# PROBIC/mSWEEP

Measured on AMD Instinct MI355X. Metric: EM iters/sec + reads×groups cells/sec, 10M reads × 5k groups, higher is better.
Workload: dtype f64

## Files before the change

### msweep_amd/csrc/host_likelihood.inc

```
namespace {

void sell_from_device(msw_core *h, const uint32_t *d_rowptr, const uint32_t *d_grp, const uint32_t *d_idx,
                      const double *cell_val = nullptr);
bool compress_dense(msw_core *h, const double *Lm, size_t ld, const double *stage, size_t G, size_t E, bool force);

}

void msw::host::reset_likelihood(msw_core *h) {
  Resident &L = h->lik;
  static_cast<LikShape &>(L) = LikShape{};
  h->solver.have_solution = false;
  h->solver.prepared = false;
  h->iperm.release();
  h->assign.drop();
  L.long_row = multilane() ? kLongRow : kLongRowOneLane;
  if (const char *lr = getenv("MSWEEP_LONG_ROW"))
    L.long_row = (uint32_t)std::min(std::max(atoi(lr), 16), (int)L.long_row);
}

namespace {

constexpr uint8_t kRGroup[64] = {0, 0, 0, 0, 1, 1, 1, 1, 1, 1, 1, 1, 0, 0, 0, 0, 1, 1, 1, 1, 0, 0,
                                 0, 0, 0, 0, 0, 0, 1, 1, 1, 1, 2, 2, 2, 2, 3, 3, 3, 3, 3, 3, 3, 3,
                                 2, 2, 2, 2, 3, 3, 3, 3, 2, 2, 2, 2, 2, 2, 2, 2, 3, 3, 3, 3};

constexpr uint8_t kRPos[64] = {0, 1, 2,  3,  0,  1,  2,  3,  4,  5,  6,  7,  4,  5,  6,  7,  8,  9,  10, 11, 8, 9,
                               10, 11, 12, 13, 14, 15, 12, 13, 14, 15, 0,  1,  2,  3,  0,  1,  2,  3,  4,  5, 6, 7,
                               4,  5,  6,  7,  8,  9,  10, 11, 8,  9,  10, 11, 12, 13, 14, 15, 12, 13, 14, 15};

struct SlotPlan {
  std::vector<uint32_t> canon, hot_rank;
  uint32_t rep_base = 0, H = 0, sentinel_slot = 0;
};
SlotPlan plan_slot_area(msw_core *h, const std::vector<uint64_t> &freq) {
  Resident &L = h->lik;
  const uint32_t n_lut = L.n_lut;
  SlotPlan sp;
  std::vector<uint32_t> used;
  for (uint32_t i = 0; i < n_lut; ++i) if (freq[i]) used.push_back(i);
  if (used.empty()) used.push_back(0);
  std::vector<uint32_t> by_freq(used);
  std::stable_sort(by_freq.begin(), by_freq.end(), [&](uint32_t a, uint32_t b) { return freq[a] > freq[b]; });
  sp.canon.assign(std::max<uint32_t>(n_lut, 1), 0);
  sp.hot_rank.assign(std::max<uint32_t>(n_lut, 1), UINT32_MAX);
  sp.sentinel_slot = used[0];
  for (uint32_t tryH : {64u, 32u, 16u, 8u, 0u}) {
    if (tryH > used.size()) continue;
    sp.H = tryH;
    sp.rep_base = sp.H ? (uint32_t)((used.size() + 15) & ~(size_t)15) : (uint32_t)used.size();
    L.n_area = sp.rep_base + 8 * sp.H;
    choose_layout(L);
    if (L.tlds && L.glds && !L.wide()) break;
  }
  bool hybrid = false;
  if (!L.tlds) {
    sp.H = 0;
    sp.rep_base = (uint32_t)used.size();
    L.n_area = (uint32_t)used.size();
    choose_layout(L);
    hybrid = choose_hybrid_layout(L, h->no_hybrid);
    if (hybrid) sp.sentinel_slot = by_freq[0];
  }
  const std::vector<uint32_t> &order = hybrid ? by_freq : used;
  std::vector<uint32_t> area_slot(L.n_area, used[0]);
  for (uint32_t e = 0; e < order.size(); ++e) area_slot[e] = order[e], sp.canon[order[e]] = e;
  for (uint32_t j = 0; j < sp.H; ++j) {
    sp.hot_rank[by_freq[j]] = j;
    for (uint32_t c = 0; c < 8; ++c) area_slot[sp.rep_base + (j >> 1) * 16 + 2 * c + (j & 1)] = by_freq[j];
  }
  L.area_slot.upload(area_slot.data(), area_slot.size(), h->stream);
  L.lut_area.alloc(L.n_area);
  hipLaunchKernelGGL(k_gather_f64, dim3((L.n_area + 255) / 256), dim3(256), 0, h->stream, L.lut.p, L.area_slot.p,
                     L.n_area, L.lut_area.p);
  L.trange.alloc(2);
  minmax_launch(1, h->stream, L.lut_area.p, (uint64_t)L.n_area, 0, L.trange.p);
  MSW_HIP(hipGetLastError());
  MSW_HIP(hipStreamSynchronize(h->stream));
  return sp;
}

void finish_sell(msw_core *h) {
  Resident &L = h->lik;
  const uint32_t wg_for_slices = (L.nslices + (kPassThreads / 64) - 1) / (kPassThreads / 64);
  L.nblk = (int)std::max<uint32_t>(1, std::min<uint32_t>(std::max(wg_for_slices, L.n_long), (uint32_t)h->n_cu));
  L.nblk_dense = 0;
  L.flavor = 0;
  L.packed_scheduled = h->pack_schedule;
  L.rows_over8 = 0;
  L.passB_rc8 = false;
  if (L.nslices && L.enc == kEncNarrow && L.cls.s0[kSliceClasses - 1] == 0) {
    DevBuf<unsigned long long> d_over;
    d_over.alloc(1);
    d_over.zero(h->stream);
    hipLaunchKernelGGL(k_rows_over, dim3(std::min<uint32_t>((L.nslices + 255) / 256, (uint32_t)h->n_cu * 8)), dim3(256), 0,
                       h->stream, L.slice_off.p, L.nslices, 8u, d_over.p);
    unsigned long long over = 0;
    MSW_HIP(hipMemcpyAsync(&over, d_over.p, sizeof over, hipMemcpyDeviceToHost, h->stream));
    MSW_HIP(hipStreamSynchronize(h->stream));
    L.rows_over8 = over;
    L.passB_rc8 = 20 * over <= L.nslots / 64;
    if (const char *e = getenv("MSWEEP_PASSB_RC")) L.passB_rc8 = atoi(e) == 8;
  }
  alloc_solve_state(L, h->solver);
  MSW_HIP(hipStreamSynchronize(h->stream));
}

template <class RP>
void upload_sell(msw_core *h, const RP *rowptr, const uint32_t *cell_grp, const uint32_t *cell_idx) {
  Resident &L = h->lik;
  const uint32_t E = L.E, G = L.G, n_lut = L.n_lut;
  const uint64_t nnz_all = rowptr[E];
  std::vector<uint64_t> freq(std::max<uint32_t>(n_lut, 1), 0);
  for (uint64_t k = 0; k < nnz_all; ++k) ++freq[cell_idx[k]];
  const SlotPlan sp = plan_slot_area(h, freq);
  const std::vector<uint32_t> &canon = sp.canon, &hot_rank = sp.hot_rank;
  const uint32_t rep_base = sp.rep_base;
  const std::vector<uint32_t> used = {sp.sentinel_slot};
  const bool wide = L.wide(), hybrid = L.hybrid();
  const int rw = wide ? 2 : 1;
  const RecDec dec = L.dec;
  const uint32_t n_hot = L.n_tab_lds;
  auto entry_of = [&](int lane, uint32_t idx) -> uint32_t {
    const uint32_t j = hot_rank[idx];
    if (lane < 0 || j == UINT32_MAX) return canon[idx];
    return rep_base + (j >> 1) * 16 + 2 * (kRPos[lane] >> 1) + (j & 1);
  };
  auto put_entry = [&](std::vector<uint32_t> &dst, size_t slot, uint32_t g, uint32_t entry, bool hot = false) {
    if (wide) {
      const uint2 r = Rec<kEncWide>::make(g, entry, dec);
      dst[2 * slot] = r.x;
      dst[2 * slot + 1] = r.y;
    } else if (hybrid) {
      dst[slot] = hot ? Rec<kEncIndex>::make_h(g, entry, dec) : Rec<kEncIndex>::make(g, entry, dec);
    } else {
      dst[slot] = Rec<kEncNarrow>::make(g, entry, dec);
    }
  };
  auto put = [&](std::vector<uint32_t> &dst, size_t slot, uint32_t g, uint32_t idx, int lane, bool hot = false) {
    put_entry(dst, slot, g, entry_of(lane, idx), hot);
  };
  std::vector<uint32_t> perm(E);
  std::vector<uint32_t> cnt_len((kLongRow + 2) * 4, 0);
  std::vector<uint8_t> ccls(E, 0);
  uint32_t n_long = 0;
  uint32_t n_class[kSliceClasses] = {};
  const bool ml = multilane();
  for (uint32_t j = 0; j < E; ++j) {
    const uint64_t len = rowptr[j + 1] - rowptr[j];
    if (hybrid && len <= 16) {
      uint32_t cc = 0;
      for (uint64_t k = rowptr[j]; k < rowptr[j + 1]; ++k) cc += canon[cell_idx[k]] >= n_hot;
      ccls[j] = (uint8_t)cold_class(cc);
    }
    if (len > (uint64_t)L.long_row) {
      ++n_long;
    } else {
      ++cnt_len[len * 4 + ccls[j]];
      ++n_class[slice_class_of((uint32_t)len, ml)];
    }
  }
  {
    std::vector<uint32_t> start((kLongRow + 2) * 4, 0);
    uint32_t pos = n_long;
    for (int len = kLongRow; len >= 0; --len)
      for (int cl = 0; cl < 4; ++cl) {
        start[len * 4 + cl] = pos;
        pos += cnt_len[len * 4 + cl];
      }
    uint32_t pl = 0;
    for (uint32_t j = 0; j < E; ++j) {
      const uint64_t len = rowptr[j + 1] - rowptr[j];
      if (len > (uint64_t)L.long_row) perm[pl++] = j;
      else perm[start[len * 4 + ccls[j]]++] = j;
    }
  }
  std::vector<uint32_t> long_ptr(n_long + 1, 0);
  for (uint32_t p = 0; p < n_long; ++p)
    long_ptr[p + 1] = long_ptr[p] + (uint32_t)(rowptr[perm[p] + 1] - rowptr[perm[p]]);
  std::vector<uint32_t> rec_long((size_t)long_ptr[n_long] * rw + 2);
  for (uint32_t p = 0; p < n_long; ++p) {
    const uint64_t b = rowptr[perm[p]];
    const uint32_t n = long_ptr[p + 1] - long_ptr[p];
    uint32_t cnt[kLongResidues] = {}, run[kLongResidues] = {};
    for (uint32_t k = 0; k < n; ++k) ++cnt[cell_grp[b + k] & (kLongResidues - 1)];
    for (uint32_t k = 0; k < n; ++k) {
      const uint32_t r = cell_grp[b + k] & (kLongResidues - 1);
      put(rec_long, (size_t)long_ptr[p] + long_cell_pos(cnt, r, run[r]++), cell_grp[b + k], cell_idx[b + k], -1);
    }
  }
  L.cls = make_slice_classes(n_class);
  const SliceClasses cls = L.cls;
  const bool schedule = h->pack_schedule;
  const uint32_t nslices = cls.s0[kSliceClasses];
  std::vector<uint32_t> slice_off(nslices + 1, 0);
  for (uint32_t s = 0; s < nslices; ++s) {
    const SliceGeo sg = slice_geo(cls, s);
    const uint32_t j0 = perm[n_long + (size_t)sg.ec0];
    const uint64_t len0 = rowptr[j0 + 1] - rowptr[j0];
    uint64_t maxlen = (len0 + (1u << sg.lgm) - 1) >> sg.lgm;
    if (!odd_slices(L.enc)) maxlen += maxlen & 1;
    const uint64_t nxt = (uint64_t)slice_off[s] + maxlen;
    if (nxt > 0xffffffffull) throw Fail("msw_core_set_csr: likelihood too large for 32-bit slice offsets");
    slice_off[s + 1] = (uint32_t)nxt;
  }
  if (hybrid && slice_off[nslices] >= (1u << kGeoHotShift))
    throw Fail("msw_core_set_csr: likelihood too large for the hybrid slot area's slice geometry");
  const size_t nslots = (size_t)slice_off[nslices] * 64;
  std::vector<uint32_t> rec((nslots + 64) * rw + 2);
  std::vector<uint8_t> slice_hot(hybrid ? nslices : 0, 0);
  {
    const int nthr = std::max(1u, std::min(32u, std::thread::hardware_concurrency()));
    std::vector<std::thread> pool;
    for (int t = 0; t < nthr; ++t) {
      pool.emplace_back([&, t] {
        std::vector<uint64_t> cells;
        std::vector<uint32_t> centry;
        std::vector<uint32_t> cbeg(65);
        std::vector<uint8_t> ctaken;
        for (uint32_t s = t; s < nslices; s += nthr) {
          const uint32_t len = slice_off[s + 1] - slice_off[s];
          const size_t base = (size_t)slice_off[s] * 64;
          cells.clear();
          centry.clear();
          const SliceGeo sg = slice_geo(cls, s);
          const uint32_t m = 1u << sg.lgm;
          for (int l = 0; l < 64; ++l) {
            cbeg[l] = (uint32_t)cells.size();
            if (((uint32_t)l >> sg.lgm) < sg.nec) {
              const uint32_t j = perm[n_long + sg.ec0 + ((uint32_t)l >> sg.lgm)];
              for (uint64_t k = rowptr[j] + ((uint32_t)l & (m - 1)); k < rowptr[j + 1]; k += m) {
                cells.push_back(((uint64_t)cell_grp[k] << 32) | cell_idx[k]);
                centry.push_back(entry_of(l, cell_idx[k]));
              }
            }
          }
          cbeg[64] = (uint32_t)cells.size();
          ctaken.assign(cells.size(), 0);
          const bool streaming = len > 16;
          for (uint32_t k0 = 0; k0 < len; k0 += 16) {
            const uint32_t nrows = std::min<uint32_t>(16, len - k0);
            uint32_t wb[64], we[64];
            for (int l = 0; l < 64; ++l) {
              wb[l] = std::min(cbeg[l] + k0, cbeg[l + 1]);
              we[l] = std::min(wb[l] + 16, cbeg[l + 1]);
            }
            uint32_t nhot = nrows;
            if (hybrid && !streaming) {
              uint32_t mc = 0;
              for (int l = 0; l < 64; ++l) {
                uint32_t cc = 0;
                for (uint32_t c = wb[l]; c < we[l]; ++c) cc += centry[c] >= n_hot;
                mc = std::max(mc, cc);
              }
              nhot = mc > (uint32_t)kColdRows ? 0u : len - mc;
              slice_hot[s] = (uint8_t)nhot;
            }
            for (uint32_t k = 0; k < nhot; ++k) {
              uint32_t rg[4][16], rs[4][16], hg[2][32];
              uint16_t at[4] = {0, 0, 0, 0};
              std::memset(rg, 0xff, sizeof rg);
              std::memset(rs, 0xff, sizeof rs);
              std::memset(hg, 0xff, sizeof hg);
              for (int li = 0; li < 64; ++li) {
                const int l = (li + (int)(k0 + k) * 7) & 63;
                const int R = kRGroup[l], C = l >> 4, H = l >> 5;
                const size_t slot = base + (size_t)(k0 + k) * 64 + l;
                int best = -1, best_score = -1;
                for (uint32_t c = wb[l]; c < we[l]; ++c) {
                  if (ctaken[c]) continue;
                  const uint32_t g = (uint32_t)(cells[c] >> 32), i = centry[c];
                  if (hybrid && !streaming && i >= n_hot) continue;
                  int score = 0;
                  if (!(at[C] >> (g & 15) & 1)) score += MSW_W_AT;
                  if (rg[R][g & 15] == UINT32_MAX || rg[R][g & 15] == g) score += MSW_W_EW;
                  if (rs[R][i & 15] == UINT32_MAX || rs[R][i & 15] == i) score += MSW_W_XT;
                  if (hg[H][g & 31] == UINT32_MAX || hg[H][g & 31] == g) score += MSW_W_E;
                  if (!schedule) score = MSW_W_AT + MSW_W_EW + MSW_W_XT + MSW_W_E;
                  if (score > best_score) {
                    best_score = score;
                    best = (int)c;
                    if (score == MSW_W_AT + MSW_W_EW + MSW_W_XT + MSW_W_E) break;
                  }
                }
                const bool hot_row = hybrid && !streaming;
                if (best < 0) {
                  put(rec, slot, G + (uint32_t)l, used[0], -1, hot_row);
                  continue;
                }
                ctaken[best] = 1;
                const uint32_t g = (uint32_t)(cells[best] >> 32), i = centry[best];
                at[C] |= (uint16_t)(1u << (g & 15));
                if (rg[R][g & 15] == UINT32_MAX) rg[R][g & 15] = g;
                if (rs[R][i & 15] == UINT32_MAX) rs[R][i & 15] = i;
                if (hg[H][g & 31] == UINT32_MAX) hg[H][g & 31] = g;
                put(rec, slot, g, (uint32_t)cells[best], l, hot_row);
              }
            }
            for (int l = 0; l < 64; ++l) {
              uint32_t c = wb[l];
              for (uint32_t k = nhot; k < nrows; ++k) {
                const size_t slot = base + (size_t)(k0 + k) * 64 + l;
                while (c < we[l] && ctaken[c]) ++c;
                if (c < we[l]) {
                  put_entry(rec, slot, (uint32_t)(cells[c] >> 32), centry[c]);
                  ++c;
                } else {
                  put(rec, slot, G + (uint32_t)l, used[0], -1);
                }
              }
            }
          }
        }
      });
    }
    for (auto &th : pool) th.join();
  }
  if (getenv("MSW_DEBUG_SCHED")) {
    uint64_t steps = 0, cyc_ew = 0, cyc_xt = 0, cyc_at = 0, cyc_e = 0;
    for (uint32_t s = 0; s < nslices; ++s) {
      const uint32_t len = slice_off[s + 1] - slice_off[s];
      const size_t base = (size_t)slice_off[s] * 64;
      for (uint32_t k = 0; k < len; ++k) {
        uint32_t vg[64], vi[64];
        for (int l = 0; l < 64; ++l) {
          const size_t slot = base + (size_t)k * 64 + l;
          if (wide) {
            const uint2 r = make_uint2(rec[2 * slot], rec[2 * slot + 1]);
            vg[l] = Rec<kEncWide>::grp(r, dec), vi[l] = Rec<kEncWide>::t_off(r, dec) >> 4;
          } else if (hybrid) {
            const bool hot = k < slice_hot[s];
            vg[l] = hot ? Rec<kEncIndex>::grp_h(rec[slot], dec) : Rec<kEncIndex>::grp(rec[slot], dec);
            vi[l] = (hot ? Rec<kEncIndex>::t_off_h(rec[slot], dec) : Rec<kEncIndex>::t_off(rec[slot], dec)) >> 4;
          } else {
            vg[l] = Rec<kEncNarrow>::grp(rec[slot], dec), vi[l] = Rec<kEncNarrow>::t_off(rec[slot], dec) >> 4;
          }
        }
        auto cyc = [&](const uint32_t *v, int ngroups, auto group_of, uint32_t nbanks, bool combine) {
          int total = 0;
          for (int gr = 0; gr < ngroups; ++gr) {
            int mx = 0;
            for (uint32_t bnk = 0; bnk < nbanks; ++bnk) {
              uint32_t seen[64]; int ns = 0;
              for (int l = 0; l < 64; ++l) if (group_of(l) == gr && (v[l] % nbanks) == bnk) {
                bool dup = false;
                if (combine) for (int q = 0; q < ns; ++q) dup |= seen[q] == v[l];
                if (!dup) seen[ns++] = v[l];
              }
              mx = std::max(mx, ns);
            }
            total += mx;
          }
          return total;
        };
        ++steps;
        cyc_ew += cyc(vg, 4, [](int l) { return (int)kRGroup[l]; }, 16, true);
        cyc_xt += cyc(vi, 4, [](int l) { return (int)kRGroup[l]; }, 16, true);
        cyc_at += cyc(vg, 4, [](int l) { return l >> 4; }, 16, false);
        cyc_e += cyc(vg, 2, [](int l) { return l >> 5; }, 32, true);
      }
    }
    fprintf(stderr, "[msw sched] steps %llu  modelled LDS cycles / wave instruction: {e,w} b128 %.2f (ideal 4)  "
                    "slot b128 %.2f (4)  atomics %.2f (4)  e_g b64 %.2f (2)\n",
            (unsigned long long)steps, (double)cyc_ew / steps, (double)cyc_xt / steps, (double)cyc_at / steps,
            (double)cyc_e / steps);
  }
  L.n_long = n_long;
  L.nslices = nslices;
  L.nslots = nslots;
  L.perm.upload(perm.data(), perm.size(), h->stream);
  L.long_ptr.upload(long_ptr.data(), long_ptr.size(), h->stream);
  L.rec_long.upload(rec_long.data(), rec_long.size(), h->stream);
  L.slice_off.upload(slice_off.data(), slice_off.size(), h->stream);
  L.rec.upload(rec.data(), rec.size(), h->stream);
  if (hybrid) L.slice_hot.upload(slice_hot.data(), std::max<size_t>(slice_hot.size(), 1), h->stream);
  finish_sell(h);
}

void set_csr_impl(msw_core *h, const uint64_t *rowptr, const uint32_t *grp, const uint32_t *cnt,
                  const double *lut, size_t lut_ld, double logzi, size_t G, size_t E) {
  Resident &L = h->lik;
// ... 208 lines not shown
```

### msweep_amd/csrc/host_pack.inc

```
namespace {

uint64_t device_scan_u32(msw_core *h, uint32_t *d, uint64_t n, DevBuf<uint32_t> &tot, DevBuf<uint64_t> &gt);

void choose_value_layout(Resident &L) {
  L.enc = kEncValue;
  L.tlds = false;
  L.n_area = 0;
  L.n_tab_lds = 0;
  L.dec.shift = 0;
  L.dec.mask = 0;
  L.dec.bhi = L.dec.bhiA = 0;
  const char *force = getenv("MSWEEP_FORCE_LDS");
  const bool want_glds = !(force && strlen(force) == 2 && force[0] == '0');
  L.glds = want_glds && pass_lds_bytes(1, 0, L.G, true, false) <= kLdsMax && passB_mode(L, true, 0, false) >= 0;
  L.gmodeB = passB_mode(L, L.glds, 0, false);
  if (L.gmodeB < 0) throw Fail("internal: no LDS configuration fits");
  if (8ull * ((uint64_t)L.G + kSentinels) >= (1ull << 31)) throw Fail("likelihood too large: group offsets exceed the record field");
}

void sell_from_device(msw_core *h, const uint32_t *d_rowptr, const uint32_t *d_grp, const uint32_t *d_idx,
                      const double *cell_val ) {
  Resident &L = h->lik;
  const uint32_t E = L.E, n_lut = L.n_lut;
  const uint64_t nnz = L.nnz;
// ... 25 lines not shown
    const size_t lds = n_lut <= 16384 ? (size_t)n_lut * sizeof(unsigned int) : 0;
    hipLaunchKernelGGL(k_slot_hist, dim3((unsigned)std::min<uint64_t>((nnz + 4095) / 4096, (uint64_t)h->n_cu * 8)), dim3(256),
                       lds, st, d_idx, nnz, n_lut, d_freq.p);
  }
  std::vector<unsigned long long> f(std::max<uint32_t>(n_lut, 1), 0);
  MSW_HIP(hipMemcpyAsync(f.data(), d_freq.p, f.size() * sizeof(unsigned long long), hipMemcpyDeviceToHost, st));
  MSW_HIP(hipStreamSynchronize(st));
  const std::vector<uint64_t> freq(f.begin(), f.end());
  sp = plan_slot_area(h, freq);
  d_canon.upload(sp.canon.data(), sp.canon.size(), st);
  d_hot.upload(sp.hot_rank.data(), sp.hot_rank.size(), st);
  }
  tm.mark("  pack: slot plan");
  DevBuf<uint32_t> key, key2, val, cnt;
  key.alloc(E);
  key2.alloc(E);
  val.alloc(E);
  L.perm.alloc(E);
  cnt.alloc(1 + kSliceClasses);
  MSW_HIP(hipMemsetAsync(cnt.p, 0, (1 + kSliceClasses) * sizeof(uint32_t), st));
  const unsigned nbe = (unsigned)std::min<size_t>(((size_t)E + 255) / 256, (size_t)h->n_cu * 16);
  hipLaunchKernelGGL(k_pack_keys, dim3(nbe), dim3(256), 0, st, d_rowptr, E, L.long_row, multilane() ? 1 : 0, d_idx,
                     L.hybrid() ? d_canon.p : (const uint32_t *)nullptr, L.n_tab_lds, key.p, val.p, cnt.p);
  size_t tmp_bytes = 0;
  MSW_HIP(prim_sort_pairs(nullptr, tmp_bytes, key.p, key2.p, val.p, L.perm.p, (size_t)E, kPackKeyBits, st));
  DevBuf<unsigned char> tmp;
  tmp.alloc(tmp_bytes);
  MSW_HIP(prim_sort_pairs(tmp.p, tmp_bytes, key.p, key2.p, val.p, L.perm.p, (size_t)E, kPackKeyBits, st));
  uint32_t counts[1 + kSliceClasses] = {};
  MSW_HIP(hipMemcpyAsync(counts, cnt.p, sizeof counts, hipMemcpyDeviceToHost, st));
  MSW_HIP(hipStreamSynchronize(st));
  tm.mark("  pack: keys + sort");
  const uint32_t n_long = counts[0];
  const uint32_t n_sell = E - n_long;
  L.cls = make_slice_classes(counts + 1);
  const uint32_t nslices = L.cls.s0[kSliceClasses];
  L.long_ptr.alloc((size_t)n_long + 1);
  L.slice_off.alloc((size_t)nslices + 1);
  MSW_HIP(hipMemsetAsync(L.long_ptr.p, 0, ((size_t)n_long + 1) * sizeof(uint32_t), st));
  MSW_HIP(hipMemsetAsync(L.slice_off.p, 0, ((size_t)nslices + 1) * sizeof(uint32_t), st));
  const uint32_t nmax = std::max(n_long, nslices);
  if (nmax)
    hipLaunchKernelGGL(k_pack_lens, dim3((nmax + 255) / 256), dim3(256), 0, st, d_rowptr, L.perm.p, n_long, nslices,
                       odd_slices(L.enc) ? 0 : 1, L.cls, L.long_ptr.p, L.slice_off.p);
  DevBuf<uint32_t> tot;
  DevBuf<uint64_t> gt;
  const uint64_t n_long_cells = device_scan_u32(h, L.long_ptr.p, (uint64_t)n_long + 1, tot, gt);
  const uint64_t n_rows = device_scan_u32(h, L.slice_off.p, (uint64_t)nslices + 1, tot, gt);
  if (n_rows > 0xffffffffull || n_long_cells > 0xffffffffull)
    throw Fail("msw_core_set_csr: likelihood too large for 32-bit slice offsets");
  uint64_t hyb_rows_max = 1ull << kGeoHotShift;
  if (const char *e = getenv("MSWEEP_HYBRID_MAX_ROWS")) hyb_rows_max = std::min<uint64_t>(hyb_rows_max, strtoull(e, nullptr, 10));
  if (L.hybrid() && n_rows >= hyb_rows_max) {
    if (h->no_hybrid) throw Fail("msw_core_set_csr: likelihood too large for the hybrid slot area's slice geometry");
    h->no_hybrid = true;
    try {
      sell_from_device(h, d_rowptr, d_grp, d_idx, cell_val);
    } catch (...) {
      h->no_hybrid = false;
      throw;
    }
    h->no_hybrid = false;
    return;
  }
  const size_t nslots = (size_t)n_rows * 64;
  if (L.hybrid()) L.slice_hot.alloc(std::max<uint32_t>(nslices, 1));
  L.rec.alloc(rec_words(L.enc, nslots + 64) + 2);
  L.rec_long.alloc(rec_words(L.enc, (size_t)n_long_cells + 64) + 2);
  MSW_HIP(hipMemsetAsync(L.rec.p + rec_words(L.enc, nslots), 0, (rec_words(L.enc, 64) + 2) * sizeof(uint32_t), st));
  MSW_HIP(hipMemsetAsync(L.rec_long.p, 0, (rec_words(L.enc, (size_t)n_long_cells + 64) + 2) * sizeof(uint32_t), st));
  tm.mark("  pack: geometry + alloc");
  const PackEnc pe{d_canon.p, d_hot.p, sp.rep_base, L.G, sp.sentinel_slot, L.dec, L.n_tab_lds, L.slice_hot.p,
                   cell_val, L.logzi};
  if (n_long) {
    auto k = L.enc == kEncValue ? k_pack_long<kEncValue>
                                 : (L.wide() ? k_pack_long<kEncWide> : (L.hybrid() ? k_pack_long<kEncIndex> : k_pack_long<kEncNarrow>));
    hipLaunchKernelGGL(k, dim3(std::min<uint32_t>(n_long, (uint32_t)h->n_cu * 32)), dim3(64), 0, st, d_rowptr, d_grp, d_idx,
                       L.perm.p, L.long_ptr.p, n_long, pe, L.rec_long.p);
  }
  if (nslices) {
    auto k = L.enc == kEncValue ? k_pack_slices<kEncValue>
                                 : (L.wide() ? k_pack_slices<kEncWide> : (L.hybrid() ? k_pack_slices<kEncIndex> : k_pack_slices<kEncNarrow>));
    hipLaunchKernelGGL(k, dim3(std::min<uint32_t>(nslices, (uint32_t)h->n_cu * 64)), dim3(64), 0, st, d_rowptr, d_grp,
                       d_idx, L.perm.p, L.slice_off.p, n_long, n_sell, nslices, L.cls, pe, h->pack_schedule ? 1 : 0, L.rec.p);
  }
  MSW_HIP(hipGetLastError());
  tm.mark("  pack: records");
  L.n_long = n_long;
  L.nslices = nslices;
  L.nslots = nslots;
  finish_sell(h);
  tm.mark("  pack: solver state");
}

uint64_t layout_hash(const Resident &L) {
  if (L.flavor != 0) throw Fail("msw_core_layout_hash: no CSR-of-ECs likelihood resident");
  uint64_t hash = 1469598103934665603ull;
  auto eat = [&](const uint32_t *d, size_t n) {
    std::vector<uint32_t> v(n);
    if (n) MSW_HIP(hipMemcpy(v.data(), d, n * sizeof(uint32_t), hipMemcpyDeviceToHost));
    const unsigned char *p = reinterpret_cast<const unsigned char *>(v.data());
    for (size_t i = 0; i < n * 4; ++i) hash = (hash ^ p[i]) * 1099511628211ull;
  };
  std::vector<uint32_t> lp(L.n_long + 1);
  MSW_HIP(hipMemcpy(lp.data(), L.long_ptr.p, lp.size() * sizeof(uint32_t), hipMemcpyDeviceToHost));
  eat(L.perm.p, L.E);
  eat(L.slice_off.p, (size_t)L.nslices + 1);
  eat(L.long_ptr.p, (size_t)L.n_long + 1);
  eat(L.rec.p, rec_words(L.enc, L.nslots));
  eat(L.rec_long.p, rec_words(L.enc, (size_t)lp[L.n_long]));
  eat(L.area_slot.p, L.n_area);
  for (int c = 0; c <= kSliceClasses; ++c) {
    const uint32_t w[2] = {L.cls.s0[c], L.cls.p0[c]};
    const unsigned char *pb = reinterpret_cast<const unsigned char *>(w);
    for (size_t i = 0; i < sizeof w; ++i) hash = (hash ^ pb[i]) * 1099511628211ull;
  }
  if (L.hybrid()) {
    std::vector<uint8_t> sh(L.nslices);
    if (L.nslices) MSW_HIP(hipMemcpy(sh.data(), L.slice_hot.p, L.nslices, hipMemcpyDeviceToHost));
    for (uint8_t b : sh) hash = (hash ^ b) * 1099511628211ull;
  }
  return hash;
}

}
```

### msweep_amd/csrc/pack_kernels.hpp

```cpp
#pragma once
#include "common.hpp"
#include "sell.hpp"

namespace msw {

__device__ __constant__ uint8_t kRGroupDev[64] = {0, 0, 0, 0, 1, 1, 1, 1, 1, 1, 1, 1, 0, 0, 0, 0, 1, 1, 1, 1, 0, 0,
                                                  0, 0, 0, 0, 0, 0, 1, 1, 1, 1, 2, 2, 2, 2, 3, 3, 3, 3, 3, 3, 3, 3,
                                                  2, 2, 2, 2, 3, 3, 3, 3, 2, 2, 2, 2, 2, 2, 2, 2, 3, 3, 3, 3};
__device__ __constant__ uint8_t kRPosDev[64] = {0,  1,  2,  3,  0,  1,  2,  3,  4,  5,  6,  7,  4,  5,  6,  7,
                                                8,  9,  10, 11, 8,  9,  10, 11, 12, 13, 14, 15, 12, 13, 14, 15,
                                                0,  1,  2,  3,  0,  1,  2,  3,  4,  5,  6,  7,  4,  5,  6,  7,
                                                8,  9,  10, 11, 8,  9,  10, 11, 12, 13, 14, 15, 12, 13, 14, 15};

__host__ __device__ inline uint32_t cold_class(uint32_t n_cold) {
  return n_cold == 0 ? 0u : (n_cold <= 2 ? 1u : (n_cold <= (uint32_t)kColdRows ? 2u : 3u));
}
constexpr uint32_t kPackKeyBits = 13;
__global__ __launch_bounds__(256) void k_pack_keys(const uint32_t *rowptr, uint32_t E, uint32_t long_row, int multilane,
                                                  const uint32_t *idx, const uint32_t *canon, uint32_t n_hot,
                                                  uint32_t *key, uint32_t *val, uint32_t *counts) {
  uint32_t mine[1 + kSliceClasses] = {};
  for (uint32_t j = blockIdx.x * blockDim.x + threadIdx.x; j < E; j += gridDim.x * blockDim.x) {
    const uint32_t b = rowptr[j], len = rowptr[j + 1] - b;
    const bool lg = len > long_row;
    uint32_t cc = 0;
    if (canon && len <= 16u)
      for (uint32_t k = 0; k < len; ++k) cc += canon[idx[b + k]] >= n_hot;
    key[j] = lg ? 0u : (1u + ((uint32_t)kLongRow - len)) * 4u + cold_class(cc);
    val[j] = j;
    const int c = lg ? 0 : 1 + slice_class_of(len, multilane != 0);
#pragma unroll
    for (int i = 0; i <= kSliceClasses; ++i) mine[i] += c == i;
  }
#pragma unroll
  for (int i = 0; i <= kSliceClasses; ++i)
    if (mine[i]) atomicAdd(&counts[i], mine[i]);
}

__global__ __launch_bounds__(256) void k_rows_over(const uint32_t *slice_off, uint32_t nslices, uint32_t limit,
                                                  unsigned long long *out) {
  unsigned long long mine = 0;
  for (uint32_t s = blockIdx.x * blockDim.x + threadIdx.x; s < nslices; s += gridDim.x * blockDim.x) {
    const uint32_t len = slice_off[s + 1] - slice_off[s];
    if (len > limit) mine += len;
  }
  if (mine) atomicAdd(out, mine);
}

__global__ __launch_bounds__(256) void k_pack_lens(const uint32_t *rowptr, const uint32_t *perm, uint32_t n_long,
                                                  uint32_t nslices, int even, SliceClasses cls, uint32_t *long_len,
                                                  uint32_t *slice_len) {
  const uint32_t i = blockIdx.x * blockDim.x + threadIdx.x;
  if (i < n_long) {
    const uint32_t j = perm[i];
    long_len[i] = rowptr[j + 1] - rowptr[j];
  }
  if (i < nslices) {
    const SliceGeo sg = slice_geo(cls, i);
    const uint32_t j = perm[n_long + (size_t)sg.ec0];
    const uint32_t len = rowptr[j + 1] - rowptr[j];
    const uint32_t rows = (len + (1u << sg.lgm) - 1u) >> sg.lgm;
    slice_len[i] = even ? rows + (rows & 1) : rows;
  }
}

__global__ __launch_bounds__(256) void k_slot_hist(const uint32_t *idx, uint64_t nnz, uint32_t n_lut,
                                                  unsigned long long *freq) {
  extern __shared__ unsigned int hist[];
  const bool lds = n_lut <= 16384;
  if (lds) {
    for (uint32_t i = threadIdx.x; i < n_lut; i += blockDim.x) hist[i] = 0;
    __syncthreads();
  }
  for (uint64_t k = (uint64_t)blockIdx.x * blockDim.x + threadIdx.x; k < nnz; k += (uint64_t)gridDim.x * blockDim.x) {
    if (lds) atomicAdd(&hist[idx[k]], 1u);
    else atomicAdd(&freq[idx[k]], 1ull);
  }
  if (lds) {
    __syncthreads();
    for (uint32_t i = threadIdx.x; i < n_lut; i += blockDim.x)
      if (hist[i]) atomicAdd(&freq[i], (unsigned long long)hist[i]);
  }
}

__global__ __launch_bounds__(256) void k_gather_f64(const double *src, const uint32_t *at, uint32_t n, double *dst) {
  const uint32_t i = blockIdx.x * blockDim.x + threadIdx.x;
  if (i < n) dst[i] = src[at[i]];
}

struct PackEnc {
  const uint32_t *canon;
  const uint32_t *hot_rank;
  uint32_t rep_base, n_groups, sentinel_slot;
  RecDec dec;
  uint32_t n_hot;
  uint8_t *slice_hot;
  const double *cell_val;
  double tnull;
};
constexpr uint32_t kPackPad = UINT32_MAX;
__device__ __forceinline__ uint32_t pack_entry(const PackEnc &pe, int lane, uint32_t idx) {
  if (pe.cell_val) return idx;
  const uint32_t j = pe.hot_rank[idx];
  if (lane < 0 || j == UINT32_MAX) return pe.canon[idx];
  return pe.rep_base + (j >> 1) * 16 + 2 * (kRPosDev[lane] >> 1) + (j & 1);
}
template <int ENC>
__device__ __forceinline__ void pack_put(uint32_t *dst, size_t slot, const PackEnc &pe, uint32_t g, uint32_t entry,
                                         bool hot = false) {
  if constexpr (ENC == kEncValue) {
    Rec<ENC>::store(dst, slot, ValRec{8u * g, entry == kPackPad ? pe.tnull : pe.cell_val[entry]});
  } else {
    if (entry == kPackPad) entry = pe.canon[pe.sentinel_slot];
    if constexpr (ENC == kEncIndex) dst[slot] = hot ? Rec<ENC>::make_h(g, entry, pe.dec) : Rec<ENC>::make(g, entry, pe.dec);
    else reinterpret_cast<typename Rec<ENC>::T *>(dst)[slot] = Rec<ENC>::make(g, entry, pe.dec);
  }
}

constexpr uint32_t kLongResidues = 32;
__host__ __device__ inline uint32_t long_cell_pos(const uint32_t *b, uint32_t r, uint32_t j) {
  uint32_t pos = 0;
  for (uint32_t q = 0; q < kLongResidues; ++q) pos += (b[q] < j ? b[q] : j) + (q < r && b[q] > j ? 1u : 0u);
  return pos;
}
template <int ENC>
__global__ __launch_bounds__(64) void k_pack_long(const uint32_t *rowptr, const uint32_t *grp, const uint32_t *idx,
                                                 const uint32_t *perm, const uint32_t *long_ptr, uint32_t n_long,
                                                 PackEnc pe, uint32_t *rec_long) {
  __shared__ uint32_t cnt[kLongResidues];
  const uint32_t lane = threadIdx.x;
  const unsigned long long lt = lane ? (~0ull >> (64 - lane)) : 0ull;
  for (uint32_t p = blockIdx.x; p < n_long; p += gridDim.x) {
    const uint32_t b = rowptr[perm[p]], n = long_ptr[p + 1] - long_ptr[p], o = long_ptr[p];
    if (lane < kLongResidues) cnt[lane] = 0;
    __syncthreads();
    for (uint32_t k = lane; k < n; k += 64) atomicAdd(&cnt[grp[b + k] & (kLongResidues - 1)], 1u);
    __syncthreads();
    uint32_t run = 0;
    for (uint32_t k0 = 0; k0 < n; k0 += 64) {
      const uint32_t k = k0 + lane;
      const bool valid = k < n;
      const uint32_t g = valid ? grp[b + k] : 0u;
      const uint32_t r = valid ? (g & (kLongResidues - 1)) : kLongResidues;
      unsigned long long mine = 0;
      uint32_t add = 0;
      for (uint32_t q = 0; q < kLongResidues; ++q) {
        const unsigned long long m = __ballot(r == q);
        if (r == q) mine = m;
        if (lane == q) add = (uint32_t)__popcll(m);
      }
      const uint32_t before = (uint32_t)__shfl((int)run, (int)(r & (kLongResidues - 1)));
      const uint32_t j = before + (uint32_t)__popcll(mine & lt);
      run += add;
      if (valid) pack_put<ENC>(rec_long, (size_t)o + long_cell_pos(cnt, r, j), pe, g, pack_entry(pe, -1, idx[b + k]));
    }
    __syncthreads();
  }
}

constexpr int kPackCells = 16;
template <int ENC>
__global__ __launch_bounds__(64) void k_pack_slices(const uint32_t *rowptr, const uint32_t *grp, const uint32_t *idx,
                                                   const uint32_t *perm, const uint32_t *slice_off, uint32_t n_long,
                                                   uint32_t n_sell, uint32_t nslices, SliceClasses cls, PackEnc pe,
                                                   int schedule, uint32_t *rec) {
  constexpr int kRowW = kPackCells + 1;
  __shared__ uint32_t cg[64 * kRowW], ce[64 * kRowW];
  struct Bank {
    uint32_t rg[4][16], rs[4][16], hg[2][32], at[4];
  };
  __shared__ Bank bk;
  auto &rg = bk.rg;
  auto &rs = bk.rs;
  auto &hg = bk.hg;
  auto &at = bk.at;
  const int lane = threadIdx.x;
  const uint32_t cand = (uint32_t)lane & 15u;
  for (uint32_t s = blockIdx.x; s < nslices; s += gridDim.x) {
    const uint32_t o = slice_off[s], L = slice_off[s + 1] - o;
    const size_t base = (size_t)o * 64;
    const SliceGeo sg = slice_geo(cls, s);
    const uint32_t m = 1u << sg.lgm, t = (uint32_t)lane & (m - 1u);
    uint32_t b = 0, mylen = 0;
    if (((uint32_t)lane >> sg.lgm) < sg.nec) {
      const uint32_t j = perm[n_long + sg.ec0 + ((uint32_t)lane >> sg.lgm)];
      const uint32_t len = rowptr[j + 1] - rowptr[j];
      b = rowptr[j] + t;
      mylen = len > t ? (len - t + m - 1u) >> sg.lgm : 0u;
    }
    const bool streaming = L > (uint32_t)kPackCells;
    if (ENC == kEncIndex && lane == 0) pe.slice_hot[s] = 0;
    const int R = kRGroupDev[lane];
    for (uint32_t k0 = 0; k0 < L; k0 += kPackCells) {
      const uint32_t nrows = min((uint32_t)kPackCells, L - k0);
      const uint32_t ncell = mylen > k0 ? min((uint32_t)kPackCells, mylen - k0) : 0u;
      uint32_t mycold = 0, coldmask = 0;
      for (uint32_t c = 0; c < ncell; ++c) {
        const uint32_t e = pack_entry(pe, lane, idx[b + (size_t)(k0 + c) * m]);
        cg[lane * kRowW + c] = grp[b + (size_t)(k0 + c) * m];
        ce[lane * kRowW + c] = e;
        mycold += e >= pe.n_hot;
        coldmask |= (uint32_t)(e >= pe.n_hot) << c;
      }
      uint32_t taken = 0, nhot = nrows;
      if constexpr (ENC == kEncIndex) {
        if (!streaming) {
          uint32_t mc = mycold;
          for (int d = 32; d; d >>= 1) mc = max(mc, (uint32_t)__shfl_xor((int)mc, d));
          nhot = mc > (uint32_t)kColdRows ? 0u : L - mc;
          if (lane == 0) pe.slice_hot[s] = (uint8_t)nhot;
        }
      }
      for (uint32_t k = 0; !schedule && k < nhot; ++k) {
        uint32_t avail = ((1u << ncell) - 1u) & ~taken;
        if (ENC == kEncIndex && !streaming) avail &= ~coldmask;
        uint32_t pick_g = pe.n_groups + lane, pick_e = kPackPad;
        if (avail) {
          const int c = __ffs((int)avail) - 1;
          taken |= 1u << c;
          pick_g = cg[lane * kRowW + c];
          pick_e = ce[lane * kRowW + c];
        }
        pack_put<ENC>(rec, base + (size_t)(k0 + k) * 64 + lane, pe, pick_g, pick_e, ENC == kEncIndex && !streaming);
      }
      for (uint32_t k = 0; schedule && k < nhot; ++k) {
        for (int w = lane; w < 196; w += 64) reinterpret_cast<uint32_t *>(&bk)[w] = w < 192 ? 0xffffffffu : 0u;
        uint32_t pick_g = pe.n_groups + lane, pick_e = kPackPad;
        __syncthreads();
        const int start = ((int)(k0 + k) * 7) & 63;
        const int sA = start < 32 ? start : 0, sB = start < 32 ? 0 : start - 32;
        const bool upper = lane >= 32;
        for (int t2 = 0; t2 < 32; ++t2) {
          const int la = (sA + t2) & 31, lb = 32 + ((sB + t2) & 31);
          const uint32_t n_a = (uint32_t)__builtin_amdgcn_readlane((int)ncell, la);
          const uint32_t t_a = (uint32_t)__builtin_amdgcn_readlane((int)taken, la);
          const uint32_t n_b = (uint32_t)__builtin_amdgcn_readlane((int)ncell, lb);
          const uint32_t t_b = (uint32_t)__builtin_amdgcn_readlane((int)taken, lb);
          const uint32_t avail_a = ((1u << n_a) - 1u) & ~t_a, avail_b = ((1u << n_b) - 1u) & ~t_b;
          if ((avail_a | avail_b) == 0) continue;
          const int R_a = __builtin_amdgcn_readlane(R, la), R_b = __builtin_amdgcn_readlane(R, lb);
          const int l = upper ? lb : la;
          const uint32_t avail = upper ? avail_b : avail_a;
          const int R_l = upper ? R_b : R_a, C_l = l >> 4, H_l = l >> 5;
          bool valid = (lane & 31) < 16 && (avail >> cand & 1u);
          uint32_t g = 0, i = 0, v_at = 0, v_rg = 0, v_rs = 0, v_hg = 0, key = 0;
          if (valid) {
            g = cg[l * kRowW + cand];
            i = ce[l * kRowW + cand];
            if (ENC == kEncIndex && !streaming && i >= pe.n_hot) valid = false;
          }
          if (valid) {
            v_at = at[C_l];
            v_rg = rg[R_l][g & 15];
            v_rs = rs[R_l][i & 15];
            v_hg = hg[H_l][g & 31];
            uint32_t score = 0;
            if (!(v_at >> (g & 15) & 1)) score += MSW_W_AT;
            if (v_rg == 0xffffffffu || v_rg == g) score += MSW_W_EW;
            if (ENC == kEncValue || v_rs == 0xffffffffu || v_rs == i) score += MSW_W_XT;
            if (v_hg == 0xffffffffu || v_hg == g) score += MSW_W_E;
            key = ((score << 4) | (15u - cand)) + 1u;
          }
          uint32_t mx = key;
          mx = max(mx, (uint32_t)__builtin_amdgcn_update_dpp(0, (int)mx, 0x111, 0xf, 0xf, false));
          mx = max(mx, (uint32_t)__builtin_amdgcn_update_dpp(0, (int)mx, 0x112, 0xf, 0xf, false));
          mx = max(mx, (uint32_t)__builtin_amdgcn_update_dpp(0, (int)mx, 0x114, 0xf, 0xf, false));
          mx = max(mx, (uint32_t)__builtin_amdgcn_update_dpp(0, (int)mx, 0x118, 0xf, 0xf, false));
          const uint32_t best_a = (uint32_t)__builtin_amdgcn_readlane((int)mx, 15);
          const uint32_t best_b = (uint32_t)__builtin_amdgcn_readlane((int)mx, 47);
          const int cb_a = 15 - (int)((best_a - 1u) & 15u), cb_b = 47 - (int)((best_b - 1u) & 15u);
          if ((best_a != 0 && lane == cb_a) || (best_b != 0 && lane == cb_b)) {
            at[C_l] = v_at | 1u << (g & 15);
            rg[R_l][g & 15] = v_rg == 0xffffffffu ? g : v_rg;
            rs[R_l][i & 15] = v_rs == 0xffffffffu ? i : v_rs;
            hg[H_l][g & 31] = v_hg == 0xffffffffu ? g : v_hg;
          }
          if (best_a != 0) {
            const uint32_t g_w = (uint32_t)__builtin_amdgcn_readlane((int)g, cb_a);
            const uint32_t i_w = (uint32_t)__builtin_amdgcn_readlane((int)i, cb_a);
            if (lane == la) {
              taken |= 1u << cb_a;
              pick_g = g_w;
              pick_e = i_w;
            }
          }
          if (best_b != 0) {
            const uint32_t g_w = (uint32_t)__builtin_amdgcn_readlane((int)g, cb_b);
            const uint32_t i_w = (uint32_t)__builtin_amdgcn_readlane((int)i, cb_b);
            if (lane == lb) {
              taken |= 1u << (cb_b - 32);
              pick_g = g_w;
              pick_e = i_w;
            }
          }
          __syncthreads();
        }
        pack_put<ENC>(rec, base + (size_t)(k0 + k) * 64 + lane, pe, pick_g, pick_e, ENC == kEncIndex && !streaming);
      }
      uint32_t c = 0;
      for (uint32_t k = nhot; k < nrows; ++k) {
        while (c < ncell && (taken >> c & 1)) ++c;
        if (c < ncell) {
          pack_put<ENC>(rec, base + (size_t)(k0 + k) * 64 + lane, pe, cg[lane * kRowW + c], ce[lane * kRowW + c]);
          ++c;
        } else {
          pack_put<ENC>(rec, base + (size_t)(k0 + k) * 64 + lane, pe, pe.n_groups + lane, kPackPad);
        }
      }
      __syncthreads();
    }
    __syncthreads();
  }
}

}
```

Measured before the change: 234300 billion.

## Add swap-based bank-conflict refinement pass to hot-row slice packing

Adds a local-search refinement after the greedy packer assigns hot rows in each slice window. For each lane column it finds the row contributing most to the modeled LDS bank and atomic conflict cost and swaps its cell with another row when that lowers the cost. The pass runs in both the host and device packers by default and can be disabled with an environment variable. The intent is fewer LDS bank conflicts in the EM likelihood kernels, at the cost of extra packing time and a larger shared-memory footprint in the pack kernel.

```diff
diff --git a/msweep_amd/csrc/bank_refine.hpp b/msweep_amd/csrc/bank_refine.hpp
--- /dev/null
+++ b/msweep_amd/csrc/bank_refine.hpp
@@ -0,0 +1,279 @@
+#pragma once
+#include <stdint.h>
+
+#if defined(__HIPCC__)
+#define MSW_REFINE_HD __host__ __device__
+#define MSW_REFINE_UNROLL _Pragma("unroll")
+#else
+#define MSW_REFINE_HD
+#define MSW_REFINE_UNROLL
+#endif
+#ifndef MSW_W_AT
+#define MSW_W_AT 8
+#define MSW_W_EW 6
+#define MSW_W_XT 4
+#define MSW_W_E 2
+#endif
+#ifndef MSW_REFINE_SWEEPS
+#define MSW_REFINE_SWEEPS 1
+#endif
+
+namespace msw {
+
+constexpr int kRefRows = 16;
+constexpr int kRefStride = 65;
+constexpr int kRefineSweeps = MSW_REFINE_SWEEPS;
+constexpr uint32_t kRefPad = 0xffffffffu;
+
+struct RefineWin {
+  uint32_t g[kRefRows * kRefStride];
+  uint32_t e[kRefRows * kRefStride];
+  uint32_t H[kRefRows][64];
+  uint8_t M[kRefRows][16];
+  uint8_t nM[kRefRows][16];
+  uint32_t D[kRefRows];
+  uint32_t X[kRefRows];
+};
+struct RefineParams {
+  uint32_t n_groups;
+  uint32_t pad_e;
+  int nh;
+  bool use_xt;
+};
+
+MSW_REFINE_HD inline int refine_rgroup(int l) { return (l >> 5) * 2 + (int)((0xF00F0FF0u >> (l & 31)) & 1u); }
+MSW_REFINE_HD inline uint32_t refine_ent(const RefineParams &p, uint32_t e) { return e == kRefPad ? p.pad_e : e; }
+MSW_REFINE_HD inline int refine_hget(const uint32_t *row, int i) { return (int)((row[i >> 2] >> (8 * (i & 3))) & 255u); }
+MSW_REFINE_HD inline void refine_hadd(uint32_t *row, int i, bool atomic) {
+#if defined(__HIP_DEVICE_COMPILE__)
+  if (atomic) {
+    atomicAdd(&row[i >> 2], 1u << (8 * (i & 3)));
+    return;
+  }
+#endif
+  (void)atomic;
+  row[i >> 2] += 1u << (8 * (i & 3));
+}
+MSW_REFINE_HD inline void refine_hsub(uint32_t *row, int i) { row[i >> 2] -= 1u << (8 * (i & 3)); }
+MSW_REFINE_HD inline int refine_og_off(int og) { return og < 12 ? og * 16 : 192 + (og - 12) * 32; }
+MSW_REFINE_HD inline int refine_og_banks(int og) { return og < 12 ? 16 : 32; }
+
+inline void refine_model_row(const uint32_t *g, const uint32_t *e, int out[4]) {
+  auto cyc = [&](const uint32_t *v, int ngroups, int kind, uint32_t nb, bool combine) {
+    int total = 0;
+    for (int gr = 0; gr < ngroups; ++gr) {
+      int mx = 0;
+      for (uint32_t b = 0; b < nb; ++b) {
+        uint32_t seen[64];
+        int ns = 0;
+        for (int l = 0; l < 64; ++l) {
+          const int mine = kind == 0 ? l >> 4 : (kind == 1 ? refine_rgroup(l) : l >> 5);
+          if (mine != gr || v[l] % nb != b) continue;
+          bool dup = false;
+          if (combine)
+            for (int q = 0; q < ns; ++q) dup |= seen[q] == v[l];
+          if (!dup) seen[ns++] = v[l];
+        }
+        mx = mx > ns ? mx : ns;
+      }
+      total += mx;
+    }
+    return total;
+  };
+  out[0] = cyc(g, 4, 0, 16, false);
+  out[1] = cyc(g, 4, 1, 16, true);
+  out[2] = cyc(e, 4, 1, 16, true);
+  out[3] = cyc(g, 2, 2, 32, true);
+}
+inline long refine_model_cost(const RefineWin &w, const RefineParams &p, int nrows) {
+  long total = 0;
+  for (int r = 0; r < nrows; ++r) {
+    uint32_t e[64];
+    int c[4];
+    for (int l = 0; l < 64; ++l) e[l] = refine_ent(p, w.e[r * kRefStride + l]);
+    refine_model_row(&w.g[r * kRefStride], e, c);
+    total += MSW_W_AT * c[0] + MSW_W_EW * c[1] + (p.use_xt ? MSW_W_XT * c[2] : 0) + MSW_W_E * c[3];
+  }
+  return total;
+}
+
+MSW_REFINE_HD inline void refine_hist_row(RefineWin &w, const RefineParams &p, int r, int j) {
+  const uint32_t *gr = &w.g[r * kRefStride], *er = &w.e[r * kRefStride];
+  const uint32_t vg = gr[j], ve = refine_ent(p, er[j]);
+  const int Rj = refine_rgroup(j);
+  bool d_ew = false, d_xt = false, d_e = false;
+  for (int q = j & 32; q < j; ++q) {
+    const bool same_r = refine_rgroup(q) == Rj;
+    const bool same_g = gr[q] == vg;
+    d_e |= same_g;
+    d_ew |= same_r && same_g;
+    d_xt |= same_r && refine_ent(p, er[q]) == ve;
+  }
+  uint32_t *h = w.H[r];
+  refine_hadd(h, (j >> 4) * 16 + (int)(vg & 15u), true);
+  if (!d_ew) refine_hadd(h, 64 + Rj * 16 + (int)(vg & 15u), true);
+  if (p.use_xt && !d_xt) refine_hadd(h, 128 + Rj * 16 + (int)(ve & 15u), true);
+  if (!d_e) refine_hadd(h, 192 + (j >> 5) * 32 + (int)(vg & 31u), true);
+}
+MSW_REFINE_HD inline void refine_max(RefineWin &w, int r, int og) {
+  const int off = refine_og_off(og), nb = refine_og_banks(og);
+  int mx = 0, n = 0;
+  for (int b = 0; b < nb; ++b) {
+    const int v = refine_hget(w.H[r], off + b);
+    if (v > mx) mx = v, n = 1;
+    else if (v == mx) ++n;
+  }
+  w.M[r][og] = (uint8_t)mx;
+  w.nM[r][og] = (uint8_t)n;
+}
+
+MSW_REFINE_HD inline int refine_cost_in(const RefineWin &w, const RefineParams &p, int l, int r, uint32_t vg, uint32_t ve,
+                                        uint32_t bits_a, uint32_t bits_v, int *exc) {
+  const uint32_t *h = w.H[r];
+  const uint32_t ag = w.g[r * kRefStride + l], ae = refine_ent(p, w.e[r * kRefStride + l]);
+  const int Rl = refine_rgroup(l);
+  int cost = 0, gain = 0;
+  MSW_REFINE_UNROLL
+  for (int o = 0; o < 4; ++o) {
+    const int og = o == 0 ? l >> 4 : (o == 1 ? 4 + Rl : (o == 2 ? 8 + Rl : 12 + (l >> 5)));
+    const uint32_t bit = o == 0 ? 0u : (o == 1 ? 1u : (o == 2 ? 2u : 4u));
+    const int wt = o == 0 ? MSW_W_AT : (o == 1 ? MSW_W_EW : (o == 2 ? (p.use_xt ? MSW_W_XT : 0) : MSW_W_E));
+    if (!wt) continue;
+    const int off = refine_og_off(og), nb = refine_og_banks(og);
+    const int bank_a = (int)((o == 2 ? ae : ag) & (uint32_t)(nb - 1)), bank_v = (int)((o == 2 ? ve : vg) & (uint32_t)(nb - 1));
+    const bool uniq = !(bits_a & bit);
+    const int mx = w.M[r][og];
+    const int mex = (uniq && refine_hget(h, off + bank_a) == mx && w.nM[r][og] == 1) ? mx - 1 : mx;
+    const int hv = refine_hget(h, off + bank_v) - (bank_v == bank_a && uniq ? 1 : 0) + ((bits_v & bit) ? 0 : 1);
+    cost += wt * (hv > mex ? hv : mex);
+    gain += wt * (mx - mex);
+  }
+  if (exc) *exc = gain;
+  return cost;
+}
+MSW_REFINE_HD inline uint32_t refine_scan(const RefineWin &w, const RefineParams &p, int l, int r, uint32_t vg, uint32_t ve, int q0,
+                                          int n) {
+  const uint32_t *gr = &w.g[r * kRefStride], *er = &w.e[r * kRefStride];
+  const int Rl = refine_rgroup(l);
+  uint32_t bits = 0;
+  for (int q = q0; q < q0 + n; ++q) {
+    if (q == l) continue;
+    const bool same_r = refine_rgroup(q) == Rl, same_g = gr[q] == vg;
+    bits |= (same_r && same_g ? 1u : 0u) | (same_r && refine_ent(p, er[q]) == ve ? 2u : 0u) | (same_g ? 4u : 0u);
+  }
+  return bits;
+}
+MSW_REFINE_HD inline void refine_or(uint32_t *word, uint32_t bits) {
+  if (!bits) return;
+#if defined(__HIP_DEVICE_COMPILE__)
+  atomicOr(word, bits);
+#else
+  *word |= bits;
+#endif
+}
+constexpr uint32_t kRefNoSwap = 0xffffffffu;
+MSW_REFINE_HD inline void refine_scan_self(RefineWin &w, const RefineParams &p, int l, int t) {
+  const int r = t >> 2;
+  if (r >= p.nh) return;
+  refine_or(&w.D[r], refine_scan(w, p, l, r, w.g[r * kRefStride + l], refine_ent(p, w.e[r * kRefStride + l]), (l & 32) + (t & 3) * 8, 8));
+}
+MSW_REFINE_HD inline uint32_t refine_worst(const RefineWin &w, const RefineParams &p, int l, int t) {
+  if (t >= p.nh || w.g[t * kRefStride + l] >= p.n_groups) return kRefNoSwap;
+  int exc = 0;
+  refine_cost_in(w, p, l, t, w.g[t * kRefStride + l], refine_ent(p, w.e[t * kRefStride + l]), w.D[t], w.D[t], &exc);
+  return exc > 0 ? ((uint32_t)(1023 - exc) << 4) | (uint32_t)t : kRefNoSwap;
+}
+MSW_REFINE_HD inline void refine_scan_pair(RefineWin &w, const RefineParams &p, int l, int r1, int t) {
+  const int r = (t & 31) >> 1, q0 = (l & 32) + (t & 1) * 16;
+  if (r >= p.nh || r == r1 || w.g[r * kRefStride + l] >= p.n_groups) return;
+  if (t < 32) refine_or(&w.X[r], refine_scan(w, p, l, r, w.g[r1 * kRefStride + l], refine_ent(p, w.e[r1 * kRefStride + l]), q0, 16));
+  else refine_or(&w.X[r], refine_scan(w, p, l, r1, w.g[r * kRefStride + l], refine_ent(p, w.e[r * kRefStride + l]), q0, 16) << 4);
+}
+MSW_REFINE_HD inline uint32_t refine_pick(const RefineWin &w, const RefineParams &p, int l, int r1, int t) {
+  if (t >= p.nh || t == r1 || w.g[t * kRefStride + l] >= p.n_groups) return kRefNoSwap;
+  const uint32_t g1 = w.g[r1 * kRefStride + l], e1 = refine_ent(p, w.e[r1 * kRefStride + l]);
+  const uint32_t g2 = w.g[t * kRefStride + l], e2 = refine_ent(p, w.e[t * kRefStride + l]);
+  const int d = refine_cost_in(w, p, l, r1, g2, e2, w.D[r1], w.X[t] >> 4, nullptr) + refine_cost_in(w, p, l, t, g1, e1, w.D[t], w.X[t] & 7u, nullptr) -
+                refine_cost_in(w, p, l, r1, g1, e1, w.D[r1], w.D[r1], nullptr) - refine_cost_in(w, p, l, t, g2, e2, w.D[t], w.D[t], nullptr);
+  return d < 0 ? ((uint32_t)(d + 32768) << 8) | (uint32_t)t : kRefNoSwap;
+}
+MSW_REFINE_HD inline void refine_apply(RefineWin &w, const RefineParams &p, int l, int r1, int r2, int t) {
+  if (t >= 8) return;
+  const int o = t & 3, r = t < 4 ? r1 : r2, c_in = t < 4 ? r2 : r1;
+  if (o == 2 && !p.use_xt) return;
+  const int Rl = refine_rgroup(l);
+  const int og = o == 0 ? l >> 4 : (o == 1 ? 4 + Rl : (o == 2 ? 8 + Rl : 12 + (l >> 5)));
+  const uint32_t bit = o == 0 ? 0u : (o == 1 ? 1u : (o == 2 ? 2u : 4u)), msk = o == 3 ? 31u : 15u;
+  const uint32_t out = o == 2 ? refine_ent(p, w.e[r * kRefStride + l]) : w.g[r * kRefStride + l];
+  const uint32_t in = o == 2 ? refine_ent(p, w.e[c_in * kRefStride + l]) : w.g[c_in * kRefStride + l];
+  const uint32_t bits_in = t < 4 ? w.X[r2] >> 4 : w.X[r2] & 7u;
+  if (!(w.D[r] & bit)) refine_hsub(w.H[r], refine_og_off(og) + (int)(out & msk));
+  if (!(bits_in & bit)) refine_hadd(w.H[r], refine_og_off(og) + (int)(in & msk), false);
+  refine_max(w, r, og);
+}
+MSW_REFINE_HD inline void refine_move(RefineWin &w, int l, int r1, int r2) {
+  const uint32_t tg = w.g[r1 * kRefStride + l], te = w.e[r1 * kRefStride + l];
+  w.g[r1 * kRefStride + l] = w.g[r2 * kRefStride + l];
+  w.e[r1 * kRefStride + l] = w.e[r2 * kRefStride + l];
+  w.g[r2 * kRefStride + l] = tg;
+  w.e[r2 * kRefStride + l] = te;
+}
+
+struct RefineSerial {
+  template <class F>
+  void each(F f) const {
+    for (int t = 0; t < 64; ++t) f(t);
+  }
+  template <class F>
+  uint32_t min_of(F f) const {
+    uint32_t best = kRefNoSwap;
+    for (int t = 0; t < 64; ++t) {
+      const uint32_t k = f(t);
+      best = k < best ? k : best;
+    }
+    return best;
+  }
+};
+
+template <class Par>
+MSW_REFINE_HD inline uint32_t refine_window(RefineWin &w, const RefineParams &p, const Par &par) {
+  if (p.nh < 2) return 0;
+  par.each([&](int t) {
+    for (int r = 0; r < p.nh; ++r) w.H[r][t] = 0;
+  });
+  par.each([&](int t) {
+    for (int r = 0; r < p.nh; ++r) refine_hist_row(w, p, r, t);
+  });
+  par.each([&](int t) {
+    for (int k = t; k < p.nh * 14; k += 64) refine_max(w, k / 14, k % 14);
+  });
+  uint32_t swaps = 0;
+  for (int sweep = 0; sweep < kRefineSweeps; ++sweep) {
+    const uint32_t before = swaps;
+    for (int l = 0; l < 64; ++l) {
+      int movable = 0;
+      for (int r = 0; r < p.nh; ++r) movable += w.g[r * kRefStride + l] < p.n_groups;
+      if (movable < 2) continue;
+      par.each([&](int t) {
+        if (t < kRefRows) w.D[t] = w.X[t] = 0;
+      });
+      par.each([&](int t) { refine_scan_self(w, p, l, t); });
+      const uint32_t worst = par.min_of([&](int t) { return t < kRefRows ? refine_worst(w, p, l, t) : kRefNoSwap; });
+      if (worst == kRefNoSwap) continue;
+      const int r1 = (int)worst & 15;
+      par.each([&](int t) { refine_scan_pair(w, p, l, r1, t); });
+      const uint32_t best = par.min_of([&](int t) { return t < kRefRows ? refine_pick(w, p, l, r1, t) : kRefNoSwap; });
+      if (best == kRefNoSwap) continue;
+      const int r2 = (int)best & 15;
+      par.each([&](int t) { refine_apply(w, p, l, r1, r2, t); });
+      par.each([&](int t) {
+        if (t == 0) refine_move(w, l, r1, r2);
+      });
+      ++swaps;
+    }
+    if (swaps == before) break;
+  }
+  return swaps;
+}
+
+}
diff --git a/msweep_amd/csrc/host_likelihood.inc b/msweep_amd/csrc/host_likelihood.inc
--- a/msweep_amd/csrc/host_likelihood.inc
+++ b/msweep_amd/csrc/host_likelihood.inc
@@ -103,6 +103,11 @@
   }
   alloc_solve_state(L, h->solver);
   MSW_HIP(hipStreamSynchronize(h->stream));
+}
+
+inline bool pack_refine_enabled() {
+  const char *e = getenv("MSWEEP_PACK_REFINE");
+  return !(e && atoi(e) == 0);
 }
 
 template <class RP>
@@ -191,6 +196,7 @@
   L.cls = make_slice_classes(n_class);
   const SliceClasses cls = L.cls;
   const bool schedule = h->pack_schedule;
+  const bool refine = pack_refine_enabled();
   const uint32_t nslices = cls.s0[kSliceClasses];
   std::vector<uint32_t> slice_off(nslices + 1, 0);
   for (uint32_t s = 0; s < nslices; ++s) {
@@ -217,6 +223,7 @@
         std::vector<uint32_t> centry;
         std::vector<uint32_t> cbeg(65);
         std::vector<uint8_t> ctaken;
+        std::unique_ptr<RefineWin> win(new RefineWin);
         for (uint32_t s = t; s < nslices; s += nthr) {
           const uint32_t len = slice_off[s + 1] - slice_off[s];
           const size_t base = (size_t)slice_off[s] * 64;
@@ -264,7 +271,6 @@
               for (int li = 0; li < 64; ++li) {
                 const int l = (li + (int)(k0 + k) * 7) & 63;
                 const int R = kRGroup[l], C = l >> 4, H = l >> 5;
-                const size_t slot = base + (size_t)(k0 + k) * 64 + l;
                 int best = -1, best_score = -1;
                 for (uint32_t c = wb[l]; c < we[l]; ++c) {
                   if (ctaken[c]) continue;
@@ -282,9 +288,9 @@
                     if (score == MSW_W_AT + MSW_W_EW + MSW_W_XT + MSW_W_E) break;
                   }
                 }
-                const bool hot_row = hybrid && !streaming;
                 if (best < 0) {
-                  put(rec, slot, G + (uint32_t)l, used[0], -1, hot_row);
+                  win->g[k * kRefStride + l] = G + (uint32_t)l;
+                  win->e[k * kRefStride + l] = kRefPad;
                   continue;
                 }
                 ctaken[best] = 1;
@@ -293,9 +299,17 @@
                 if (rg[R][g & 15] == UINT32_MAX) rg[R][g & 15] = g;
                 if (rs[R][i & 15] == UINT32_MAX) rs[R][i & 15] = i;
                 if (hg[H][g & 31] == UINT32_MAX) hg[H][g & 31] = g;
-                put(rec, slot, g, (uint32_t)cells[best], l, hot_row);
+                win->g[k * kRefStride + l] = g;
+                win->e[k * kRefStride + l] = i;
               }
             }
+            const RefineParams rp{G, entry_of(-1, used[0]), (int)nhot, true};
+            if (schedule && refine) refine_window(*win, rp, RefineSerial());
+            const bool hot_row = hybrid && !streaming;
+            for (uint32_t k = 0; k < nhot; ++k)
+              for (int l = 0; l < 64; ++l)
+                put_entry(rec, base + (size_t)(k0 + k) * 64 + l, win->g[k * kRefStride + l],
+                          refine_ent(rp, win->e[k * kRefStride + l]), hot_row);
             for (int l = 0; l < 64; ++l) {
               uint32_t c = wb[l];
               for (uint32_t k = nhot; k < nrows; ++k) {
diff --git a/msweep_amd/csrc/host_pack.inc b/msweep_amd/csrc/host_pack.inc
--- a/msweep_amd/csrc/host_pack.inc
+++ b/msweep_amd/csrc/host_pack.inc
@@ -131,7 +131,7 @@
     auto k = L.enc == kEncValue ? k_pack_slices<kEncValue>
                                  : (L.wide() ? k_pack_slices<kEncWide> : (L.hybrid() ? k_pack_slices<kEncIndex> : k_pack_slices<kEncNarrow>));
     hipLaunchKernelGGL(k, dim3(std::min<uint32_t>(nslices, (uint32_t)h->n_cu * 64)), dim3(64), 0, st, d_rowptr, d_grp,
-                       d_idx, L.perm.p, L.slice_off.p, n_long, n_sell, nslices, L.cls, pe, h->pack_schedule ? 1 : 0, L.rec.p);
+                       d_idx, L.perm.p, L.slice_off.p, n_long, n_sell, nslices, L.cls, pe, h->pack_schedule ? (pack_refine_enabled() ? 2 : 1) : 0, L.rec.p);
   }
   MSW_HIP(hipGetLastError());
   tm.mark("  pack: records");
diff --git a/msweep_amd/csrc/pack_kernels.hpp b/msweep_amd/csrc/pack_kernels.hpp
--- a/msweep_amd/csrc/pack_kernels.hpp
+++ b/msweep_amd/csrc/pack_kernels.hpp
@@ -1,6 +1,7 @@
 #pragma once
 #include "common.hpp"
 #include "sell.hpp"
+#include "bank_refine.hpp"
 
 namespace msw {
 
@@ -159,6 +160,22 @@
 }
 
 constexpr int kPackCells = 16;
+static_assert(kPackCells == kRefRows && kPackPad == kRefPad, "bank_refine.hpp works on the packer's windows");
+struct RefineWave {
+  template <class F>
+  __device__ void each(F f) const {
+    f((int)threadIdx.x);
+    __syncthreads();
+  }
+  template <class F>
+  __device__ uint32_t min_of(F f) const {
+    uint32_t k = f((int)threadIdx.x);
+    for (int d = 32; d; d >>= 1) k = min(k, (uint32_t)__shfl_xor((int)k, d));
+    k = (uint32_t)__builtin_amdgcn_readfirstlane((int)k);
+    __syncthreads();
+    return k;
+  }
+};
 template <int ENC>
 __global__ __launch_bounds__(64) void k_pack_slices(const uint32_t *rowptr, const uint32_t *grp, const uint32_t *idx,
                                                    const uint32_t *perm, const uint32_t *slice_off, uint32_t n_long,
@@ -170,6 +187,7 @@
     uint32_t rg[4][16], rs[4][16], hg[2][32], at[4];
   };
   __shared__ Bank bk;
+  __shared__ RefineWin win;
   auto &rg = bk.rg;
   auto &rs = bk.rs;
   auto &hg = bk.hg;
@@ -295,7 +313,16 @@
           }
           __syncthreads();
         }
-        pack_put<ENC>(rec, base + (size_t)(k0 + k) * 64 + lane, pe, pick_g, pick_e, ENC == kEncIndex && !streaming);
+        win.g[k * kRefStride + lane] = pick_g;
+        win.e[k * kRefStride + lane] = pick_e;
+      }
+      if (schedule) {
+        __syncthreads();
+        const RefineParams rp{pe.n_groups, ENC == kEncValue ? 0u : pe.canon[pe.sentinel_slot], (int)nhot, ENC != kEncValue};
+        if (schedule == 2) refine_window(win, rp, RefineWave());
+        for (uint32_t k = 0; k < nhot; ++k)
+          pack_put<ENC>(rec, base + (size_t)(k0 + k) * 64 + lane, pe, win.g[k * kRefStride + lane], win.e[k * kRefStride + lane],
+                        ENC == kEncIndex && !streaming);
       }
       uint32_t c = 0;
       for (uint32_t k = nhot; k < nrows; ++k) {
```

New measurement: 233200 billion. About the same (-0.5%).
